# ChenFengTsai/dreamerv3-torch

Hardware: AMD Instinct MI355X
Metric: imagination-steps/sec (higher is better)
Workload: dtype f32; 1 GPU; cfg2: dmc_vision 64x64x3 synthetic replay, RSSM deter=512 hidden=512 stoch=32x32, continuous actor (6), imag_gradient dynamics, batch 16 x seq 64 per GPU, horizon 15; one step = full Dreamer._train update (world model + actor + critic fwd/bwd, gradient all-reduce, 3x clip+Adam); global_batch=16, seq_len=64, horizon=15, parallelism=dp1

## Files before the change

dreamerv3-torch_amd/csrc/fusedops.hip:

```cpp
#include "dv3_common.h"

namespace dv3 {

typedef float f32x4 __attribute__((ext_vector_type(4)));
typedef float f32x4u __attribute__((ext_vector_type(4), aligned(4)));

struct OLParams {
  const int* idx;
  int S, D;
  const float* x2;
  long ldx2;
  int A2;
  const float* WT;
  long ldw;
  const float* base;
  long ldbase;
  float* pre;
  long ldpre;
  const float* gamma;
  const float* beta;
  float* y;
  long ldy;
  float* mean;
  float* rstd;
// ... 195 lines not shown
      const float d = p.pre[r * p.ldpre + c] - mean;
      q += d * d;
    }
    const float rstd = rsqrtf(block_sum_256(q, red) * inv_n + kLnEps);
    for (int c = tid; c < p.N; c += 256) {
      const float t = (p.pre[r * p.ldpre + c] - mean) * rstd * p.gamma[c] + p.beta[c];
      p.y[r * p.ldy + c] = p.act ? siluf_(t) : t;
    }
    if (tid == 0) {
      if (p.mean) p.mean[r] = mean;
      if (p.rstd) p.rstd[r] = rstd;
    }
  }
}

struct AHParams {
  const float* pre;
  long ldpre;
  const float* gamma;
  const float* beta;
  float* y;
  long ldy;
  float* mean;
  float* rstd;
  const float* Wm;
  const float* bm;
  const float* Ws;
  const float* bs;
  float* out_m;
  float* out_s;
// ... 273 lines not shown
      ldpre < N || (base && ldbase < N))
    return DV3_ERR_ARG;
  if (y && (!gamma || !beta || ldy < N)) return DV3_ERR_ARG;
  OLParams p{idx, S, D, x2, ldx2, A2, WT, ldw, base, ldbase, pre, ldpre, gamma, beta, y, ldy, mean, rstd, M, N, act};
  hipStream_t s = (hipStream_t)stream;
  const bool vec = (N % 256 == 0) && N <= 1024 && (ldw % 4 == 0) && (ldpre % 4 == 0) && (!base || ldbase % 4 == 0) &&
                   (!y || ldy % 4 == 0);
  if (vec) {
    const dim3 grid(cap_grid(M, 1, 32768)), block(256);
    switch (N / 256) {
      case 1: hipLaunchKernelGGL((onehot_linear_ln_vec_kernel<1>), grid, block, 0, s, p); break;
      case 2: hipLaunchKernelGGL((onehot_linear_ln_vec_kernel<2>), grid, block, 0, s, p); break;
      case 3: hipLaunchKernelGGL((onehot_linear_ln_vec_kernel<3>), grid, block, 0, s, p); break;
      default: hipLaunchKernelGGL((onehot_linear_ln_vec_kernel<4>), grid, block, 0, s, p); break;
    }
  } else {
    hipLaunchKernelGGL(onehot_linear_ln_generic_kernel, dim3(cap_grid(M, 1, 16384)), dim3(256), 0, s, p);
  }
  return (int)hipGetLastError();
}

extern "C" int dv3_onehot_sample_linear_ln_fwd(const float* logit, const float* noise,
                                               const unsigned long long* rng_state, unsigned long long rng_offset,
                                               float* onehot, int* idx, const int* forced, unsigned int* flips,
                                               float unimix, int mode, const float* next_first, const float* init,
                                               const int* init_idx, float* next_out, int* next_idx, int S,
                                               const float* x2, long ldx2, int A2, const float* WT, long ldw,
                                               float* pre, long ldpre, const float* gamma, const float* beta, float* y,
                                               long ldy, float* mean, float* rstd, long M, int N, int act,
                                               void* stream) {
// ... 94 lines not shown
```

dreamerv3-torch_amd/dv3hip/engine.py:

```python
from __future__ import annotations

from dataclasses import dataclass
from typing import Dict, List, Optional

import torch

from . import _dev, ops

F32 = torch.float32


_FUSE_BLEND = _dev.flag("DV3_FUSE_BLEND", True)
_FUSE_SAMPLE = _dev.flag("DV3_FUSE_SAMPLE", True)
_GATHER_OBS = _dev.flag("DV3_GATHER_OBS", True)
_FUSE_SAMPLE_IN = _dev.flag("DV3_FUSE_SAMPLE_IN", True)
_FUSE_CARRY = _dev.flag("DV3_FUSE_CARRY", True)
_FUSE_SCAN_ROW = _dev.flag("DV3_FUSE_SCAN_ROW", True)
_FUSE_SCAN_LN = _dev.flag("DV3_FUSE_SCAN_LN", True)
_FUSE_SCAN_LNBWD = _dev.flag("DV3_FUSE_SCAN_LNBWD", True)
_FUSE_SCAN_CS = _dev.flag("DV3_FUSE_SCAN_CS", True)
_DEFER_CONV_WGRAD = _dev.flag("DV3_DEFER_CONV_WGRAD", True)
_FUSE_SCAN_GRUBWD = _dev.flag("DV3_FUSE_SCAN_GRUBWD", True)


class Lanes:

    _by_dev: Dict[str, "Lanes"] = {}

    @classmethod
    def get(cls, device):
        key = str(torch.device(device))
        if key not in cls._by_dev:
            try:
                cls._by_dev[key] = Lanes(device, _dev.value("DV3_LANES_SCAN_CUS", 0))
            except (RuntimeError, ValueError) as e:
                import sys

# ... 328 lines not shown

def v2(t: torch.Tensor, cols: int) -> torch.Tensor:
    return t.reshape(-1, cols)


def dense_ln_fwd(L: PDenseLN, x1, x2, pre, mean, rstd, y, *, accumulate_pre=False):
    ops.gemm(x1, L.W, pre, A2=x2, accumulate=accumulate_pre)
    ops.ln_act_fwd(pre, L.g, L.b, y, mean, rstd, act=True)


def dense_ln_bwd_pre(L: PDenseLN, dy, pre, mean, rstd, dpre, *, wgrad: bool):
    ops.ln_act_bwd(dy, pre, L.g, L.b, mean, rstd, dpre, _g(L.g) if wgrad else None, _g(L.b) if wgrad else None,
                   act=True)


def lin_wgrad(W, dY, x1, x2=None):
    k1 = x1.shape[1]
    gW = _g(W)
    ops.gemm(dY, x1, gW[:, :k1] if x2 is not None else gW, transA=True, transB=False, accumulate=True)
    if x2 is not None:
        ops.gemm(dY, x2, gW[:, k1:], transA=True, transB=False, accumulate=True)


class MLPEngine:

    def __init__(self, name: str, P: PMLP, ws: Workspace):
        self.name, self.P, self.ws = name, P, ws
        self.total = 0

    def _bufs(self, total):
        P, ws, nm = self.P, self.ws, self.name
        self.total = total
        acts = []
        for i, L in enumerate(P.layers):
# ... 49 lines not shown
                           None if onehot else out2[rs], head["action"], head["ent"], noise=head.get("noise"),
                           rng=head.get("rng"), eps_out=head.get("eps_out"), act_idx=head.get("act_idx"),
                           forced=head.get("forced"), flips=head.get("flips"), min_std=head.get("min_std", 0.1),
                           max_std=head.get("max_std", 1.0), unimix=head.get("unimix", 0.01), onehot=onehot)
            return h1, out[rs], None if onehot else out2[rs]
        o = o2 = None
        if out is not None:
            o = out[rs]
            ops.gemm(h1, P.out.W, o, A2=h2, bias=P.out.b)
        if out2 is not None:
            o2 = out2[rs]
            ops.gemm(h1, P.out2.W, o2, bias=P.out2.b)
        return h1, o, o2

    def backward(self, x1, x2, rows: slice, dout=None, dout2=None, *, wgrad: bool, dx1=None, dx2=None,
                 acc_dx=False, dh=None, defer=None):
        P, ws, nm = self.P, self.ws, self.name
        acts, _, _ = self._bufs(self.total)
        R = x1.shape[0]
        n_layers = len(P.layers)
        h = acts[-1][3][rows] if n_layers else x1
        first = True
        if dh is not None:
            first = False
        else:
            dh = ws.get(f"{nm}.dh", (R, h.shape[1]))
        for lin, d in ((P.out, dout), (P.out2, dout2)):
            if lin is None or d is None:
                continue
            ops.gemm(d, lin.W, dh, transB=False, accumulate=not first)
            first = False
# ... 1 lines not shown
                def _head_wgrad(lin=lin, d=d, h=h):
                    lin_wgrad(lin.W, d, h)
                    if lin.b is not None:
                        ops.colsum(d, _g(lin.b), accumulate=True)
                (defer.append if defer is not None else (lambda f: f()))(_head_wgrad)
        if first:
            raise ValueError("MLP backward without any upstream gradient")
        dy = dh
        for i in reversed(range(n_layers)):
            L = P.layers[i]
            pre, mean, rstd, _ = acts[i]
            xin1, xin2 = (acts[i - 1][3][rows], None) if i > 0 else (x1, x2)
            dpre = ws.get(f"{nm}.dpre{i}", (R, pre.shape[1]))
            dense_ln_bwd_pre(L, dy, pre[rows], mean[rows], rstd[rows], dpre, wgrad=wgrad)
            if wgrad:
                def _wg(L=L, dpre=dpre, xin1=xin1, xin2=xin2):
                    lin_wgrad(L.W, dpre, xin1, xin2)
                (defer.append if defer is not None else (lambda f: f()))(_wg)
            if i > 0:
                dprev = ws.get(f"{nm}.dy{i - 1}", (R, xin1.shape[1]))
                ops.gemm(dpre, L.W, dprev, transB=False)
                dy = dprev
            else:
                k1 = x1.shape[1]
                if dx1 is not None:
                    ops.gemm(dpre, L.W[:, :k1] if x2 is not None else L.W, dx1, transB=False, accumulate=acc_dx)
                if dx2 is not None and x2 is not None:
                    ops.gemm(dpre, L.W[:, k1:], dx2, transB=False, accumulate=acc_dx)


def _scan_bandwidth_bound(De: int, Hd: int, B: int) -> bool:
    gru_weight_bytes = 4 * 3 * De * (Hd + De)
# ... 279 lines not shown
                                      gd[t - 1] if t > 0 else None, dstoch0, ddeter0)
        side.join()
        ops.gemm(v2(dx3pre, Hd), P.obs_out.W[:, De:], v2(dembed, E), transB=False)
        dpl = v2(dpl_out, SW)

        def _scan_wgrads():
            if prior_inline:
                _prior_wgrads()
            lin_wgrad(P.obs.W, dpl, v2(x3, Hd))
            ops.colsum(dpl, _g(P.obs.b), accumulate=True)
            lin_wgrad(P.obs_out.W, v2(dx3pre, Hd), v2(deter, De), v2(self._embed, E))
            lin_wgrad(P.gru.W, v2(dgpre, 3 * De), v2(x1, Hd), v2(din, De))
            lin_wgrad(P.img_in.W, v2(dx1pre, Hd), v2(sin, SD), v2(ain, A))
            self.init_state_bwd(dstoch0, ddeter0)

        side.run([_scan_wgrads], chain=False)
        return side

    def pack_img_in(self, defer=None, name="rssm.img_in_wt"):
        W = self.P.img_in.W
        wt = self.ws.get(name, (W.shape[1], W.shape[0]))
        if defer is not None:
            defer.append((W, wt))
        else:
            ops.transpose2d(W, wt)
        return wt

    def img_step_fwd(self, stoch, deter, action, bufs, *, noise=None, rng=None, sample=True, forced=None,
                     flips=None, idx=None, idx_out=None, wcat=None, head=True):
        P = self.P
        M = stoch.shape[0]
# ... 152 lines not shown
            ops.ln_act_bwd(dy if last else dy.view(R, Co), pre.view(R, Co), L.g, L.b, mean, rstd, dpre.view(R, Co),
                           _g(L.g), _g(L.b), act=True, chw_group=OH * OH if last else 0)
            ops.conv_s2_wgrad(dpre, x, _g(L.W))
            if i > 0:
                wpt = ws.get(f"enc.wpt{i}", (4, Ci, 4 * Co))
                ops.pack_conv_weight(L.W, wpt, transposed=True)
                dx = ws.get(f"enc.dy{i - 1}", x.shape)
                ops.convT_s2_fwd(dpre, wpt, dx, Ci=Co, Co=Ci)
                dy = dx


class ConvDecoderEngine:
    def __init__(self, lin: PLin, layers: List[PConvLayer], ws: Workspace, minres=4):
        self.lin, self.L, self.ws, self.minres = lin, layers, ws, minres

    def forward(self, x1, x2):
        ws = self.ws
        R = x1.shape[0]
        E = self.lin.W.shape[0]
        mr = self.minres
        C0 = E // (mr * mr)
        h0 = ws.get("dec.h0", (R, mr, mr, C0))
        ops.gemm(x1, self.lin.W, h0.view(R, E), A2=x2, bias=self.lin.b)
        self._x = (x1, x2)
        self._acts = []
        x, H = h0, mr
        for i, L in enumerate(self.L):
            Ci, Co = L.W.shape[0], L.W.shape[1]
            OH = 2 * H
            c3 = L.g is None and Co == 3 and Ci in ops.C3_WIDTHS
            if not c3:
                wpt = ws.get(f"dec.wpt{i}", (4, Co, 4 * Ci))
                ops.pack_conv_weight(L.W, wpt, transposed=True)
            if L.g is not None:
                pre = ws.get(f"dec.pre{i}", (R, OH, OH, Co))
                ops.convT_s2_fwd(x, wpt, pre, Ci=Ci, Co=Co)
                rows = R * OH * OH
                mean, rstd = ws.get(f"dec.m{i}", (rows,)), ws.get(f"dec.r{i}", (rows,))
# ... 30 lines not shown
                    run(lambda dpre=dpre, L=L, rows=rows, Co=Co: ops.colsum(dpre.view(rows, Co), _g(L.bias),
                                                                         accumulate=True))
            (run if _DEFER_CONV_WGRAD else (lambda f: f()))(lambda x=x, dpre=dpre, L=L: ops.conv_s2_wgrad(x, dpre, _g(L.W)))
            dx = ws.get(f"dec.dx{i}", x.shape)
            if Co == 3 and Ci in ops.C3_WIDTHS:
                ops.conv_s2_c3_fwd(dpre, L.W, dx, CW=Ci)
            else:
                wp = ws.get(f"dec.wp{i}", (Ci, 16 * Co))
                ops.pack_conv_weight(L.W, wp, transposed=False)
                ops.conv_s2_fwd(dpre, wp, dx, Ci=Co, Co=Ci)
            dy = dx
        R = dy.shape[0]
        E = self.lin.W.shape[0]
        dh0 = dy.view(R, E)
        x1, x2 = self._x

        def _lin_wg():
            lin_wgrad(self.lin.W, dh0, x1, x2)
            ops.colsum(dh0, _g(self.lin.b), accumulate=True)

        run(_lin_wg)
        k1 = x1.shape[1]
        ops.gemm(dh0, self.lin.W[:, :k1], dx1, transB=False, accumulate=acc_dx)
        ops.gemm(dh0, self.lin.W[:, k1:], dx2, transB=False, accumulate=acc_dx)


class EnsembleEngine:

    def __init__(self, name: str, bucket, layers: int, ws: Workspace, *, std: float, scale: float = 1.0, log: bool = True):
        if bucket.members < 2 or layers < 1:
            raise ValueError("EnsembleEngine: needs at least 2 members (the unbiased std) and 1 trunk layer")
        self.name, self.bucket, self.L, self.ws = name, bucket, int(layers), ws
        self.K = bucket.members
# ... 102 lines not shown
```

dreamerv3-torch_amd/dv3hip/graph.py:

```python
from __future__ import annotations

from typing import Dict

import numpy as np
import torch

from . import _dev, _lib, ops


class CaptureRefused(RuntimeError):
    """The HIP runtime (or torch) refused stream capture / graph instantiation.  The ONLY condition under which the
    runners fall back to eager launches; shape bugs, a non-zero return code of a dv3 kernel (DV3Error) or an
    asynchronous HIP fault propagate to the caller."""


_CAPTURE_REFUSALS = (
    "hiperrorstreamcapture", "cudaerrorstreamcapture", "hiperrorcapturedevent", "hiperrorgraphexecupdatefailure",
    "operation not permitted when stream is capturing", "operation failed due to a previous error during capture",
    "operation would result in a merge of separate capture sequences",
    "capture was not ended in the same stream as it began", "capturing stream has unjoined work",
    "dependency created on uncaptured work in another stream",
    "operation would make the legacy stream depend on a capturing blocking stream",
    "operation not permitted on an event last recorded in a capturing stream",
    "attempt to terminate a thread-local capture sequence from another thread",
# ... 141 lines not shown
    @staticmethod
    def _launch(g, stream, lane, trace):
        if trace is None:
            g.replay()
            return
        a, b = torch.cuda.Event(enable_timing=True), torch.cuda.Event(enable_timing=True)
        a.record(stream)
        g.replay()
        b.record(stream)
        trace.append((lane, a, b))


_PIPE_PLAN = dict(on=_dev.flag("DV3_PIPE", True), a_split=_dev.value("DV3_PIPE_A_SPLIT", 0) or None,
                  c_split=_dev.value("DV3_PIPE_C_SPLIT", 0) or None, defer=_dev.value("DV3_PIPE_DEFER", "auto", str),
                  late=_dev.flag("DV3_PIPE_LATE", True), mode=_dev.value("DV3_PIPE_MODE", "auto", str),
                  defer_split=_dev.value("DV3_PIPE_DEFER_SPLIT", 0) or None)


class PhaseRecorder:

    def __init__(self, pool, device, lanes, lane_of, first_label, optional=()):
        self.pool, self.device, self.lanes = pool, device, lanes
        self.lane_of, self.first, self.optional = lane_of, first_label, set(optional)
        self.segments = []
        self._cur = None

    def _begin(self, label):
        g = torch.cuda.CUDAGraph()
        kw = dict(pool=self.pool, capture_error_mode="thread_local")
        lane = self.lane_of(label)
        if lane != "main":
# ... 355 lines not shown
        wm, beh = self.wm, self.beh
        dev = next(iter(self._static.values())).device
        lanes = engine.Lanes.get(dev)
        plan = self.pipe_plan
        rng_wm, rng_beh = ops.PhasedRng(dev), ops.PhasedRng(dev)
        key_dev = wm.dynamics.W.device
        lane_wm = lambda lb: {"wm.fscan": "scan", "wm.fscan2": "scan", "wm.rscan": "scan", "wm.rscan2": "scan",
                              "wm.defer": "side"}.get(lb, "main")
        lane_beh = lambda lb: "side" if lb.startswith(("bh.A", "bh.C")) else "main"
        mode = self._pipe_mode()
        if plan.get("defer", "auto") == "auto":
            plan["defer"] = "post" if wm._config.imag_gradient in ("dynamics", "both") else "side"
        if mode == "staged" and plan["defer"] != "side":
            lane_wm = lambda lb: {"wm.fscan": "scan", "wm.fscan2": "scan", "wm.rscan": "scan", "wm.rscan2": "scan"}.get(lb, "main")
        if mode == "lanes":
            lane_wm = lambda lb: "side" if lb == "wm.defer" else "scan"
            lane_beh = lambda lb: "side"
        opt_cuts = [f"bh.A@{plan['a_split']}"] if plan.get("a_split") else []
        opt_cuts += [f"bh.C@{plan['c_split']}"] if plan.get("c_split") else []
        cap = {}
        pool_w, pool_b = torch.cuda.graph_pool_handle(), torch.cuda.graph_pool_handle()
        w_cuts = [f"wm.defer@{plan['defer_split']}"] if (plan.get("defer_split") and mode == "lanes") else []
        with tools.rng_override(key_dev, rng_wm):
            W = PhaseRecorder(pool_w, dev, lanes, lane_wm, "wm.pre", optional=w_cuts).record(
                lambda: wm.train_fwd_bwd(self._static), at_end=rng_wm.finish_phase)
            gw = torch.cuda.CUDAGraph()

            def wopt():
                cap["post"], cap["ctx"], cap["m1"] = wm.train_opt(allreduce=False)

            _capture(gw, wopt, pool=pool_w)
        with tools.rng_override(key_dev, rng_beh):
            B = PhaseRecorder(pool_b, dev, lanes, lane_beh, "bh.start", optional=opt_cuts).record(
                lambda: beh.train_fwd_bwd(cap["post"]), at_end=rng_beh.finish_phase)
            gb = torch.cuda.CUDAGraph()
            _capture(gb, lambda: cap.update(beh_out=beh.train_opt(allreduce=False)), pool=pool_b)
        stride = rng_wm.taken + rng_beh.taken
        rng_wm.stride.fill_(stride), rng_beh.stride.fill_(stride)
        mk = lambda: torch.cuda.Event(blocking=True)
        self._pipe = dict(W=W.segments, B=B.segments, wopt=gw, bopt=gb, cap=cap, rng_wm=rng_wm, rng_beh=rng_beh,
                          lanes=lanes, entered=False, shared=tools.default_rng(key_dev), mode=mode,
                          ev={k: mk() for k in ("tail", "fork1", "q1", "mid", "fork2", "q2")},
                          ev2={k: (mk() if k == "mid" else torch.cuda.Event()) for k in ("load", "start", "mid", "defer", "wopt")},
                          ring=[mk(), mk()])

    def _pipe_enter(self):
        P = self._pipe
        sh = P["shared"]
        sh.commit()
        P["rng_beh"].state.copy_(sh.state)
        P["rng_wm"].state.copy_(sh.state)
        P["rng_wm"].state[1:2].add_(P["rng_beh"].taken)
        P["entered"] = True

    def _pipe_leave(self):
        P = self._pipe
        if P.get("lanes_running"):
            cur = torch.cuda.current_stream()
# ... 25 lines not shown
            ev["mid"].synchronize()
        self._load(data)
        ev["load"].record(cur)
        X.wait_event(ev["load"])
        if first:
            Y.wait_event(ev["load"])
        else:
            Y.wait_event(ev["wopt"])
        run(B, ["bh.start"], Y)
        ev["start"].record(Y)
        run(W, ["wm.pre"], X)
        run(B, [lb for lb in B if lb != "bh.start"], Y)
        X.wait_event(ev["start"])
        run(W, ["wm.fscan", "wm.fscan2", "wm.mid"], X)
        ev["mid"].record(X)
        run(W, ["wm.rscan", "wm.rscan2", "wm.post"] + [lb for lb in W if lb.startswith("wm.defer@")], X)
        with torch.cuda.stream(Y):
            self.beh._actor_opt.bucket.allreduce()
            self.beh._value_opt.bucket.allreduce()
            self._traced("bh.opt", P["bopt"])
            self._sink(1, P["cap"]["beh_out"][-1])
        Y.wait_event(ev["mid"])
        run(W, ["wm.defer"], Y)
        ev["defer"].record(Y)
        X.wait_event(ev["defer"])
        with torch.cuda.stream(X):
            self.wm._model_opt.bucket.allreduce()
            self._traced("wm.opt", P["wopt"])
            self._sink(0, P["cap"]["m1"])
        ev["wopt"].record(X)
        ring[it % 2].record(X)
        P["lanes_running"] = True

    def _traced(self, label, g):
        trace = self._pipe_trace
        if trace is None:
            g.replay()
            return
# ... 276 lines not shown
```

dreamerv3-torch_amd/dv3hip/ops.py:

```python
from __future__ import annotations

from typing import Optional

import torch

from . import _dev, _lib

F32 = torch.float32


def _stream() -> int:
    return torch.cuda.current_stream().cuda_stream


def _ptr(t: Optional[torch.Tensor]) -> int:
    return 0 if t is None else t.data_ptr()


def _f32(t: torch.Tensor, name: str) -> None:
    if not isinstance(t, torch.Tensor) or not t.is_cuda or t.dtype != F32:
        raise TypeError(f"{name}: expected a CUDA/HIP float32 tensor, got "
                        f"{type(t).__name__} {getattr(t, 'dtype', None)} {getattr(t, 'device', None)}")


# ... 1503 lines not shown
        _contig(gamma, "gamma"), _contig(beta, "beta")
        if (My, Ny) != (M, N) or gamma.numel() != N or beta.numel() != N:
            raise ValueError("y / LN affine shape mismatch")
        for t, nm in ((mean, "mean"), (rstd, "rstd")):
            if t is not None:
                _contig(t, nm)
                if t.numel() != M:
                    raise ValueError(nm + " size mismatch")
    _call("dv3_onehot_linear_ln_fwd", _ptr(idx), S, int(D), _ptr(x2), ldx2, A2, _ptr(WT), ldw, _ptr(base), ldbase,
          _ptr(pre), ldpre, _ptr(gamma), _ptr(beta), _ptr(y), ldy, _ptr(mean), _ptr(rstd), M, N, int(act), _stream(),
          key="dv3_onehot_linear_ln_fwd" + (f"[{M}x{N},S={S}]" if PROFILE.by_shape else ""),
          flops=2.0 * M * N * (S * D + A2), nbytes=4.0 * M * N * (S + 2))
    return y if y is not None else pre


def sample_linear_ln_ok(S, D, N) -> bool:
    return D == 32 and S <= 32 and N % 256 == 0 and N <= 1024


def onehot_sample_linear_ln(logit, out, *, next_first, init, init_idx, next_out, next_idx, WT, x2, pre, gamma, beta, y,
                            mean, rstd, noise=None, rng=None, idx=None, forced=None, flips=None, unimix=0.01,
                            mode=False, act=True):
    if logit.dim() != 3 or logit.shape[2] != 32:
        raise ValueError("logit must be [M,S,32]")
    M, S, D = logit.shape
    Kw, N, ldw = _rows2d(WT, "WT")
    Mp, Np, ldpre = _rows2d(pre, "pre")
    My, Ny, ldy = _rows2d(y, "y")
    Mx, A2, ldx2 = _rows2d(x2, "x2") if x2 is not None else (M, 0, 0)
    if not sample_linear_ln_ok(S, D, N) or (Mp, Np) != (M, N) or (My, Ny) != (M, N) or Mx != M or Kw != S * D + A2:
# ... 312 lines not shown
```

dreamerv3-torch_amd/models.py:

```python
from __future__ import annotations

import copy

import numpy as np
import torch
from torch import nn

import networks
import tools
from dv3hip import _dev
from dv3hip import engine as E
from dv3hip import ops
from dv3hip.params import ParamBucket

to_np = lambda x: x.detach().cpu().numpy()
_FUSED_IMAG = _dev.flag("DV3_FUSED_IMAG", True)
_STACK_DETER = _dev.flag("DV3_STACK_DETER", True)


import weakref

_BEHAVIORS = weakref.WeakKeyDictionary()
_RUNNERS = weakref.WeakKeyDictionary()

# ... 205 lines not shown
            ops.gauss_kl_fwd(out["post_mean"], out["post_std"], out["prior_mean"], out["prior_std"], kl, ent_p, ent_q)
        else:
            ops.kl_fwd(out["post_logit"], out["prior_logit"], kl, ent_p, ent_q, unimix=dyn._unimix_ratio)
        lanes_pay = rssm.lanes_pay(heavy_side=bool(self.heads["decoder"].cnn_shapes))
        E.SideStream.host_sync_point(lanes_pay)

        up = 1.0 / TB
        dec = self.heads["decoder"]
        acc = ws.zeros("wm.acc", (8 + len(dec.mlp_shapes),))
        gs, gd = ws.get("wm.gs", (T, B, SD)), ws.get("wm.gd", (T, B, De))
        wrote = False
        deferred = []
        grad_heads = cfg.grad_heads
        if dec.cnn_shapes:
            dec_eng = dec._cnn.engine
            recon = dec_eng.forward(ps, dt)
            limg = ws.get("wm.loss_img", (TB,))
            drecon = ws.get("wm.drecon", recon.shape)
            ops.mse_image(recon, st["image"], limg, drecon, upstream=up, perm=(B, T))
            ops.dot_accumulate(limg, acc[1:2], scale=up)
            dec_eng.backward(drecon, gs.view(TB, SD), gd.view(TB, De), acc_dx=False, defer=deferred)
            self._defer_heads_from = len(deferred)
            wrote = True
            if "decoder" not in grad_heads:
                gs.zero_(), gd.zero_()
        if dec.mlp_shapes:
            mdec = dec._mlp
            deng = mdec.engine_for(".wm")
            h, _, _ = deng.forward(ps, dt)
            dh = ws.zeros("wm.dec_dh", h.shape)
            for ki, (k, shp) in enumerate(dec.mlp_shapes.items()):
# ... 520 lines not shown
                       mix=getattr(cfg, "imag_gradient_mix", 0.0))
        R = H1N

        def _critic():
            inv = 1.0 / H1N
            up_v = ops.scale_neg(weights.view(HN)[:R], g("bh.up_v", (R,)), inv)
            lp, lp2 = g("bh.lp_v", (R,)), g("bh.lp_v2", (R,))
            dvl = g("bh.dv_logits", (R, 255))
            ops.disc_logprob_fwd(v_logits[:R], target.view(R), lp)
            ops.dot_accumulate(lp, acc[1:2], w=up_v)
            ops.disc_logprob_bwd(v_logits[:R], target.view(R), up_v, dvl)
            if cfg.critic["slow_target"]:
                ops.disc_logprob_fwd(v_logits[:R], slow.view(R), lp2)
                ops.dot_accumulate(lp2, acc[1:2], w=up_v)
                ops.disc_logprob_bwd(v_logits[:R], slow.view(R), up_v, dvl, accumulate=True)
            veng.backward(fs[:R], fd[:R], slice(0, R), dout=dvl, wgrad=True)

        E.Cuts.mark("bh.B@critic")
        side = E.SideStream(fs.device)
        side.run([_critic], chain=False)
        E.Cuts.mark("bh.B@dyn")
        daction = g("bh.daction", (H, N, A))
        if not reinforce:
            dreward, dcl = g("bh.dreward", (H, N)), g("bh.dcont", (H, N))
            ops.lambda_return_bwd(dtarget, value, c_logit.view(H, N), target, dreward, dcl, gamma=cfg.discount,
                                  lam=cfg.discount_lambda)
            gs, gd = g("bh.gs", (H, N, SD)), g("bh.gd", (H, N, De))
            rows = slice(N, HN)
            g_act = None
            if ens is not None:
                gs.view(HN, SD)[rows].zero_()
# ... 39 lines not shown
                ops.axpby(g_act.reshape(H, N, A).contiguous(), daction, 1.0, 1.0)
                R = HN
        dmean, dstd = g("bh.dmean", (R, A)), g("bh.dstd", (R, A))
        if normal:
            ops.actor_normal_bwd(a_mean[:R], a_std[:R], dmean, dstd, eps=im["eps"].view(HN, A)[:R],
                                 action=action.view(HN, A)[:R], daction=None if reinforce else daction.view(HN, A)[:R],
                                 dent=dent.view(HN)[:R], dlogp=dlogp.view(HN)[:R] if use_logp else None,
                                 min_std=cfg.actor["min_std"], max_std=cfg.actor["max_std"], logp_of_sample=use_logp)
        else:
            if not reinforce:
                ops.onehot_st_bwd(a_mean[:R], daction.view(HN, A)[:R], dmean, unimix=cfg.actor["unimix_ratio"])
            ops.onehot_ent_logp_bwd(a_mean[:R], action.view(HN, A)[:R], dent.view(HN)[:R],
                                    dlogp.view(HN)[:R] if use_logp else None, dmean,
                                    unimix=cfg.actor["unimix_ratio"], accumulate=not reinforce)
            dstd = None
        im["actor"].backward(fs[:R], fd[:R], slice(0, R), dout=dmean, dout2=dstd, wgrad=True)
        side.join()
        ops.dot_accumulate(ent.view(HN), acc[2:3], scale=1.0 / HN)
        metrics = {}
        groups = [(value[:-1], "value", None, None), (target, "target", None, None), (reward, "imag_reward", None, None),
                  (action if normal else torch.argmax(action, dim=-1).float(), "imag_action", None, None)]
        if cfg.imag_gradient == "both":
            metrics["imag_gradient_mix"] = cfg.imag_gradient_mix
        if cfg.reward_EMA:
            scale = torch.clip(ema[1:2] - ema[0:1], min=1.0)
            groups.append((target, "normed_target", ema[0:1], scale))
            metrics["EMA_005"], metrics["EMA_095"] = ema[0], ema[1]
        metrics.update(tools.tensorstats_many(groups))
        metrics["actor_entropy"] = acc[2]
        self.ema_to_wire()
        self._last = dict(reward=reward, value=value, target=target, weights=weights, disc=disc, slow=slow)
# ... 8 lines not shown
```

include/dv3hip.h:

```cpp
#ifndef DV3HIP_H_
#define DV3HIP_H_

#ifdef __cplusplus
extern "C" {
#endif

#define DV3_ERR_ARG 10001

int dv3_version(void);
int dv3_dev_switches(void);

int dv3_gemm_f32(int transA, int transB, int M, int N, int K, const float* A, long lda, const float* A2,
                 long lda2, int K1, const float* B, long ldb, float* C, long ldc, const float* bias,
                 int accumulate, int tile, void* stream);

int dv3_gemm_split_f32(int M, int N, int K, const float* A, long lda, const float* B, long ldb, float* C, long ldc,
                       int accumulate, float* C2, long ldc2, int nsplit, int accumulate2, void* stream);

int dv3_gemm_tn_grouped_f32(int n, const float* const* A, const long* lda, const float* const* B, const long* ldb,
                            float* const* C, const long* ldc, const int* M, const int* N, const int* K,
                            const int* accumulate, void* stream);

int dv3_gemm_sample_f32(int M, int N, int K, const float* A, long lda, const float* A2, long lda2, int K1,
                        const float* B, long ldb, float* C, long ldc, const float* bias, const float* noise,
// ... 193 lines not shown

int dv3_onehot_linear_ln_fwd(const int* idx, int S, int D, const float* x2, long ldx2, int A2, const float* WT,
                             long ldw, const float* base, long ldbase, float* pre, long ldpre, const float* gamma,
                             const float* beta, float* y, long ldy, float* mean, float* rstd, long M, int N, int act,
                             void* stream);
int dv3_actor_head_fwd(const float* pre, long ldpre, const float* gamma, const float* beta, float* y, long ldy,
                       float* mean, float* rstd, const float* Wm, const float* bm, const float* Ws, const float* bs,
                       float* out_m, float* out_s, const float* noise, const unsigned long long* rng_state,
                       unsigned long long rng_offset, float* eps_out, float* action, float* entropy, int* act_idx,
                       const int* forced, unsigned int* flips, long M, int U, int A, float min_std, float max_std,
                       float unimix, int onehot, void* stream);
int dv3_transpose2d(const float* src, long lds, int R, int C, float* dst, long ldd, void* stream);
int dv3_transpose2d_many(int njobs, const unsigned long long* jobs_host, void* stream);
int dv3_onehot_to_idx(const float* onehot, int* idx, long R, int D, void* stream);

int dv3_ens_gemm_f32(int members, int transA, int transB, int M, int N, int K, const float* A, long lda,
                     long strideA, const float* B, long ldb, long strideB, float* C, long ldc, long strideC,
                     const float* bias, long strideBias, int accumulate, void* stream);
int dv3_ens_ln_act_fwd(const float* x, long ldx, const float* gamma, const float* beta, long strideG, float* y,
                       long ldy, float* mean, float* rstd, int members, int M, int N, void* stream);
int dv3_ens_ln_act_bwd(const float* dy, long lddy, const float* x, long ldx, const float* gamma, const float* beta,
                       long strideG, const float* mean, const float* rstd, float* dx, long lddx, float* dgamma,
                       float* dbeta, int members, int M, int N, void* stream);
int dv3_ens_colsum(const float* x, long ldx, long strideX, float* out, long strideOut, int members, int M, int N,
                   int accumulate, void* stream);
int dv3_ens_regress_loss(const float* pre, const float* target, long ldt, float* dpre, float* loss, float* ws,
                         int members, int M, int W, float std, void* stream);
int dv3_ens_disag_fwd(const float* h, long ldh, long strideH, const float* w, long ldw, long strideW,
                      const float* bias, long strideBias, float* mu, float* part, float* disag, float* reward,
                      long ldr, int members, int M, int W, int U, float scale, int use_log, void* stream);
// ... 12 lines not shown
```

Before: 1.187 million imagination-steps/s.

## Use sparse one-hot kernels for decoder linear and actor/critic weight gradients

Adds a kernel that computes weight gradients for one-hot stochastic inputs by scatter-adding dY rows into per-category LDS bins, with a row-chunked fold. The dense GEMM over a mostly-zero one-hot matrix goes away. The decoder's first linear layer now uses a gathered one-hot forward through a new wide kernel plus a transposed weight copy. The pipeline also moves the RSSM scan weight-gradient segment to the side lane and sets the default defer split to 6. This brings extra workspace and a transpose, and the new paths are more complex.

```diff
diff --git a/dreamerv3-torch_amd/csrc/fusedops.hip b/dreamerv3-torch_amd/csrc/fusedops.hip
--- a/dreamerv3-torch_amd/csrc/fusedops.hip
+++ b/dreamerv3-torch_amd/csrc/fusedops.hip
@@ -233,6 +233,31 @@
   }
 }
 
+__global__ __launch_bounds__(256) void onehot_linear_wide_kernel(OLParams p) {
+  const int c = blockIdx.y * 1024 + 4 * threadIdx.x;
+  if (c >= p.N) return;
+  constexpr int MAXB = 16;
+  for (long r = blockIdx.x; r < p.M; r += gridDim.x) {
+    f32x4 acc = (f32x4){0.f, 0.f, 0.f, 0.f};
+    if (p.base) acc = *reinterpret_cast<const f32x4u*>(p.base + r * p.ldbase + c);
+    for (int s0 = 0; s0 < p.S; s0 += MAXB) {
+      f32x4 t[MAXB];
+#pragma unroll
+      for (int u = 0; u < MAXB; ++u) {
+        const int s = s0 + u;
+        t[u] = (f32x4){0.f, 0.f, 0.f, 0.f};
+        if (s < p.S) t[u] = *reinterpret_cast<const f32x4u*>(p.WT + (long)(s * p.D + p.idx[r * p.S + s]) * p.ldw + c);
+      }
+#pragma unroll
+      for (int u = 0; u < MAXB; ++u)
+        if (s0 + u < p.S) acc += t[u];
+    }
+    for (int a = 0; a < p.A2; ++a)
+      acc += p.x2[r * p.ldx2 + a] * *reinterpret_cast<const f32x4u*>(p.WT + (long)(p.S * p.D + a) * p.ldw + c);
+    *reinterpret_cast<f32x4u*>(p.pre + r * p.ldpre + c) = acc;
+  }
+}
+
 struct AHParams {
   const float* pre;
   long ldpre;
@@ -536,6 +561,9 @@
       case 3: hipLaunchKernelGGL((onehot_linear_ln_vec_kernel<3>), grid, block, 0, s, p); break;
       default: hipLaunchKernelGGL((onehot_linear_ln_vec_kernel<4>), grid, block, 0, s, p); break;
     }
+  } else if (!y && N > 1024 && N % 4 == 0 && ldw % 4 == 0 && ldpre % 4 == 0 && (!base || ldbase % 4 == 0)) {
+    hipLaunchKernelGGL(onehot_linear_wide_kernel, dim3(cap_grid(M, 1, 16384), (unsigned)((N + 1023) / 1024)), dim3(256), 0,
+                       s, p);
   } else {
     hipLaunchKernelGGL(onehot_linear_ln_generic_kernel, dim3(cap_grid(M, 1, 16384)), dim3(256), 0, s, p);
   }
diff --git a/dreamerv3-torch_amd/csrc/onehotops.hip b/dreamerv3-torch_amd/csrc/onehotops.hip
--- /dev/null
+++ b/dreamerv3-torch_amd/csrc/onehotops.hip
@@ -0,0 +1,202 @@
+#include "dv3_common.h"
+
+namespace dv3 {
+
+typedef float f32x4 __attribute__((ext_vector_type(4)));
+
+constexpr int kOwGroups = 8;
+constexpr int kOwRowChunk = 1024;
+constexpr int kOwRows = 4;
+constexpr int kOwBatches = 8;
+
+struct OWParams {
+  const int* idx;
+  int S;
+  const float* dY;
+  long lddy;
+  float* out;
+  long ldo;
+  long chunk_stride;
+  long R;
+  int U;
+  int accumulate;
+};
+
+template <int CPT>
+__device__ __forceinline__ int ow_slot(int j, int d) {
+  return d * (64 * CPT) + ((j + d) & 63) * CPT;
+}
+
+template <int CPT>
+__global__ __launch_bounds__(256) void onehot_wgrad_kernel(OWParams p) {
+  typedef float VT __attribute__((ext_vector_type(CPT)));
+  constexpr int CW = 64 * CPT, GW = kOwGroups / 4, RU = kOwRows, PF = kOwBatches;
+  extern __shared__ __attribute__((aligned(16))) float ow_bins[];
+  const int wave = __builtin_amdgcn_readfirstlane(threadIdx.x >> 6), l = threadIdx.x & 63;
+  const int s0 = blockIdx.y * kOwGroups + wave * GW;
+  if (s0 >= p.S) return;
+  const int ng = (p.S - s0 < GW) ? p.S - s0 : GW;
+  float* mine = ow_bins + wave * GW * 32 * CW;
+  for (int i = l * 4; i < GW * 32 * CW; i += 256) *reinterpret_cast<f32x4*>(mine + i) = (f32x4){0.f, 0.f, 0.f, 0.f};
+  const long r0 = (long)blockIdx.z * kOwRowChunk;
+  const long r1 = (r0 + kOwRowChunk < p.R) ? r0 + kOwRowChunk : p.R;
+  const float* __restrict__ dy = p.dY + (long)blockIdx.x * CW + l * CPT;
+  const int* __restrict__ ix = p.idx + s0;
+
+  const int lk = (l & (RU * GW - 1)) / GW, lg = (l % GW < ng) ? l % GW : ng - 1;
+  const long nfull = (r1 - r0) / (RU * PF) * (RU * PF);
+  VT xq[PF][RU];
+  int iq[PF];
+  if (nfull > 0) {
+#pragma unroll
+    for (int b = 0; b < PF; ++b) {
+#pragma unroll
+      for (int k = 0; k < RU; ++k) xq[b][k] = *reinterpret_cast<const VT*>(dy + (r0 + b * RU + k) * p.lddy);
+      iq[b] = ix[(r0 + b * RU + lk) * p.S + lg];
+    }
+  }
+  long r = r0;
+  for (; r < r0 + nfull; r += RU * PF) {
+#pragma unroll
+    for (int b = 0; b < PF; ++b) {
+    VT x[RU];
+    int id[RU][GW];
+#pragma unroll
+    for (int k = 0; k < RU; ++k) {
+      x[k] = xq[b][k];
+#pragma unroll
+      for (int g = 0; g < GW; ++g) id[k][g] = __builtin_amdgcn_readlane(iq[b], k * GW + g) & 31;
+    }
+    {
+      const long rn = r + (long)(PF + b) * RU;
+#pragma unroll
+      for (int k = 0; k < RU; ++k) {
+        const long rr = (rn + k < r0 + nfull) ? rn + k : r0 + nfull - 1;
+        xq[b][k] = *reinterpret_cast<const VT*>(dy + rr * p.lddy);
+      }
+      const long ri = (rn + lk < r0 + nfull) ? rn + lk : r0 + nfull - 1;
+      iq[b] = ix[ri * p.S + lg];
+    }
+    __builtin_amdgcn_sched_barrier(0);
+    VT bv[GW][RU], v[GW][RU];
+#pragma unroll
+    for (int g = 0; g < GW; ++g)
+#pragma unroll
+      for (int k = 0; k < RU; ++k) bv[g][k] = *reinterpret_cast<const VT*>(mine + g * 32 * CW + ow_slot<CPT>(l, id[k][g]));
+#pragma unroll
+    for (int g = 0; g < GW; ++g)
+#pragma unroll
+      for (int k = 0; k < RU; ++k) {
+        VT src = bv[g][k];
+#pragma unroll
+        for (int j = 0; j < k; ++j)
+          if (id[j][g] == id[k][g]) src = v[g][j];
+        v[g][k] = src + x[k];
+      }
+#pragma unroll
+    for (int g = 0; g < GW; ++g)
+#pragma unroll
+      for (int k = 0; k < RU; ++k) *reinterpret_cast<VT*>(mine + g * 32 * CW + ow_slot<CPT>(l, id[k][g])) = v[g][k];
+    __builtin_amdgcn_sched_barrier(0);
+    }
+  }
+  for (; r < r1; ++r) {
+    const VT xr = *reinterpret_cast<const VT*>(dy + r * p.lddy);
+    for (int g = 0; g < ng; ++g) {
+      VT* b = reinterpret_cast<VT*>(mine + g * 32 * CW + ow_slot<CPT>(l, ix[r * p.S + g] & 31));
+      *b = *b + xr;
+    }
+  }
+
+  float* out = p.out + (long)blockIdx.z * p.chunk_stride;
+  const int d = l & 31, h = l >> 5;
+  constexpr int WB = 16;
+  for (int g = 0; g < ng; ++g) {
+    const float* bin = mine + g * 32 * CW;
+    for (int c0 = h; c0 < CW; c0 += 2 * WB) {
+      float vsum[WB], old[WB];
+      float* o[WB];
+#pragma unroll
+      for (int j = 0; j < WB; ++j) {
+        const int c = c0 + 2 * j;
+        vsum[j] = bin[ow_slot<CPT>(c / CPT, d) + c % CPT];
+        o[j] = out + ((long)blockIdx.x * CW + c) * p.ldo + (long)(s0 + g) * 32 + d;
+        old[j] = 0.f;
+      }
+      if (p.accumulate) {
+#pragma unroll
+        for (int j = 0; j < WB; ++j) old[j] = *o[j];
+      }
+#pragma unroll
+      for (int j = 0; j < WB; ++j) *o[j] = old[j] + vsum[j];
+    }
+  }
+}
+
+__global__ __launch_bounds__(256) void onehot_wgrad_fold_kernel(const float* __restrict__ part, int chunks, long chunk_stride,
+                                                                float* gW, long ldw, int U, int SD, int accumulate) {
+  const long n = (long)U * SD;
+  for (long i = (long)blockIdx.x * 256 + threadIdx.x; i < n; i += (long)gridDim.x * 256) {
+    const long u = i / SD;
+    const int j = (int)(i - u * SD);
+    float* o = gW + u * ldw + j;
+    float acc = accumulate ? *o : 0.f;
+    for (int z = 0; z < chunks; ++z) acc += part[z * chunk_stride + i];
+    *o = acc;
+  }
+}
+
+static int ow_chunks(long R) { return (int)((R + kOwRowChunk - 1) / kOwRowChunk); }
+static bool ow_shape_ok(long R, int S, int D, int U) {
+  return D == 32 && S > 0 && U > 0 && U % 64 == 0 && R > 0 && ow_chunks(R) <= 65535 && (S + kOwGroups - 1) / kOwGroups <= 65535;
+}
+
+template <int CPT>
+static int ow_launch(const OWParams& p, dim3 grid, hipStream_t s) {
+  constexpr size_t lds = sizeof(float) * kOwGroups * 32 * 64 * CPT;
+  if (lds > 64 * 1024) {
+    static unsigned long long seen[4];
+    if (dv3_first_on_device(seen)) {
+      const hipError_t e = hipFuncSetAttribute(reinterpret_cast<const void*>(&onehot_wgrad_kernel<CPT>),
+                                               hipFuncAttributeMaxDynamicSharedMemorySize, (int)lds);
+      if (e != hipSuccess) return (int)e;
+    }
+  }
+  hipLaunchKernelGGL((onehot_wgrad_kernel<CPT>), grid, dim3(256), lds, s, p);
+  return (int)hipGetLastError();
+}
+
+}
+
+using namespace dv3;
+
+extern "C" int dv3_onehot_wgrad_row_chunk(void) { return kOwRowChunk; }
+
+extern "C" int dv3_onehot_wgrad_chunks(long R, int S, int D, int U) { return ow_shape_ok(R, S, D, U) ? ow_chunks(R) : 0; }
+
+extern "C" int dv3_onehot_wgrad_f32(const int* idx, int S, int D, const float* dY, long lddy, float* gW, long ldw, long R,
+                                    int U, int accumulate, float* ws, long ws_floats, void* stream) {
+  if (R <= 0) return 0;
+  if (!idx || !dY || !gW || D <= 0 || S <= 0 || U <= 0 || lddy < U || ldw < (long)S * D) return DV3_ERR_ARG;
+  if (!ow_shape_ok(R, S, D, U)) return DV3_ERR_ARG;
+  const int chunks = ow_chunks(R);
+  const long SD = (long)S * D, part = (long)U * SD;
+  if (chunks > 1 && (!ws || ws_floats < chunks * part)) return DV3_ERR_ARG;
+  hipStream_t s = (hipStream_t)stream;
+  OWParams p{idx, S, dY, lddy, gW, ldw, 0, R, U, accumulate ? 1 : 0};
+  if (chunks > 1) {
+    p.out = ws;
+    p.ldo = SD;
+    p.chunk_stride = part;
+    p.accumulate = 0;
+  }
+  const bool two = (U % 128 == 0) && (lddy % 2 == 0) && ((uintptr_t)dY % 8 == 0);
+  const dim3 grid((unsigned)(U / (two ? 128 : 64)), (unsigned)((S + kOwGroups - 1) / kOwGroups), (unsigned)chunks);
+  const int e = two ? ow_launch<2>(p, grid, s) : ow_launch<1>(p, grid, s);
+  if (e != 0 || chunks == 1) return e;
+  long blocks = (part + 255) / 256;
+  if (blocks > 16384) blocks = 16384;
+  hipLaunchKernelGGL(onehot_wgrad_fold_kernel, dim3((unsigned)blocks), dim3(256), 0, s, ws, chunks, part, gW, ldw, U,
+                     (int)SD, accumulate ? 1 : 0);
+  return (int)hipGetLastError();
+}
diff --git a/dreamerv3-torch_amd/dv3hip/engine.py b/dreamerv3-torch_amd/dv3hip/engine.py
--- a/dreamerv3-torch_amd/dv3hip/engine.py
+++ b/dreamerv3-torch_amd/dv3hip/engine.py
@@ -21,6 +21,7 @@
 _FUSE_SCAN_CS = _dev.flag("DV3_FUSE_SCAN_CS", True)
 _DEFER_CONV_WGRAD = _dev.flag("DV3_DEFER_CONV_WGRAD", True)
 _FUSE_SCAN_GRUBWD = _dev.flag("DV3_FUSE_SCAN_GRUBWD", True)
+_ONEHOT_WGRAD = _dev.flag("DV3_ONEHOT_WGRAD", True)
 
 
 class Lanes:
@@ -379,10 +380,14 @@
                    act=True)
 
 
-def lin_wgrad(W, dY, x1, x2=None):
+def lin_wgrad(W, dY, x1, x2=None, idx=None, D=0):
     k1 = x1.shape[1]
     gW = _g(W)
-    ops.gemm(dY, x1, gW[:, :k1] if x2 is not None else gW, transA=True, transB=False, accumulate=True)
+    g1 = gW[:, :k1] if x2 is not None else gW
+    if idx is not None and _ONEHOT_WGRAD and ops.onehot_wgrad_ok(idx.shape[0], idx.shape[1], D, dY.shape[1]):
+        ops.onehot_wgrad(idx, D, dY, g1, accumulate=True)
+    else:
+        ops.gemm(dY, x1, g1, transA=True, transB=False, accumulate=True)
     if x2 is not None:
         ops.gemm(dY, x2, gW[:, k1:], transA=True, transB=False, accumulate=True)
 
@@ -462,7 +467,7 @@
         return h1, o, o2
 
     def backward(self, x1, x2, rows: slice, dout=None, dout2=None, *, wgrad: bool, dx1=None, dx2=None,
-                 acc_dx=False, dh=None, defer=None):
+                 acc_dx=False, dh=None, defer=None, idx=None, D=0):
         P, ws, nm = self.P, self.ws, self.name
         acts, _, _ = self._bufs(self.total)
         R = x1.shape[0]
@@ -494,8 +499,8 @@
             dpre = ws.get(f"{nm}.dpre{i}", (R, pre.shape[1]))
             dense_ln_bwd_pre(L, dy, pre[rows], mean[rows], rstd[rows], dpre, wgrad=wgrad)
             if wgrad:
-                def _wg(L=L, dpre=dpre, xin1=xin1, xin2=xin2):
-                    lin_wgrad(L.W, dpre, xin1, xin2)
+                def _wg(L=L, dpre=dpre, xin1=xin1, xin2=xin2, idx=idx if i == 0 else None):
+                    lin_wgrad(L.W, dpre, xin1, xin2, idx, D)
                 (defer.append if defer is not None else (lambda f: f()))(_wg)
             if i > 0:
                 dprev = ws.get(f"{nm}.dy{i - 1}", (R, xin1.shape[1]))
@@ -805,7 +810,9 @@
             lin_wgrad(P.img_in.W, v2(dx1pre, Hd), v2(sin, SD), v2(ain, A))
             self.init_state_bwd(dstoch0, ddeter0)
 
+        Cuts.mark("wm.swg@side")
         side.run([_scan_wgrads], chain=False)
+        Cuts.mark("wm.post@enc")
         return side
 
     def pack_img_in(self, defer=None, name="rssm.img_in_wt"):
@@ -988,14 +995,31 @@
     def __init__(self, lin: PLin, layers: List[PConvLayer], ws: Workspace, minres=4):
         self.lin, self.L, self.ws, self.minres = lin, layers, ws, minres
 
-    def forward(self, x1, x2):
+    def pack_onehot(self, SD: int, defer=None):
+        W = self.lin.W
+        wt = self.ws.get("dec.wt", (SD, W.shape[0]))
+        if defer is not None:
+            defer.append((W[:, :SD], wt))
+        else:
+            ops.transpose2d(W[:, :SD], wt)
+        return wt
+
+    def forward(self, x1, x2, idx=None, D=0):
         ws = self.ws
         R = x1.shape[0]
         E = self.lin.W.shape[0]
         mr = self.minres
         C0 = E // (mr * mr)
         h0 = ws.get("dec.h0", (R, mr, mr, C0))
-        ops.gemm(x1, self.lin.W, h0.view(R, E), A2=x2, bias=self.lin.b)
+        if idx is not None and _ONEHOT_WGRAD:
+            SD = idx.shape[1] * D
+            hv = h0.view(R, E)
+            ops.gemm(x2, self.lin.W[:, SD:], hv, bias=self.lin.b)
+            ops.onehot_linear_ln(idx, D, ws.get("dec.wt", (SD, E)), hv, base=hv)
+        else:
+            idx = None
+            ops.gemm(x1, self.lin.W, h0.view(R, E), A2=x2, bias=self.lin.b)
+        self._idx = (idx, D)
         self._x = (x1, x2)
         self._acts = []
         x, H = h0, mr
@@ -1056,9 +1080,10 @@
         E = self.lin.W.shape[0]
         dh0 = dy.view(R, E)
         x1, x2 = self._x
+        idx, D = self._idx
 
         def _lin_wg():
-            lin_wgrad(self.lin.W, dh0, x1, x2)
+            lin_wgrad(self.lin.W, dh0, x1, x2, idx, D)
             ops.colsum(dh0, _g(self.lin.b), accumulate=True)
 
         run(_lin_wg)
diff --git a/dreamerv3-torch_amd/dv3hip/graph.py b/dreamerv3-torch_amd/dv3hip/graph.py
--- a/dreamerv3-torch_amd/dv3hip/graph.py
+++ b/dreamerv3-torch_amd/dv3hip/graph.py
@@ -179,7 +179,8 @@
 _PIPE_PLAN = dict(on=_dev.flag("DV3_PIPE", True), a_split=_dev.value("DV3_PIPE_A_SPLIT", 0) or None,
                   c_split=_dev.value("DV3_PIPE_C_SPLIT", 0) or None, defer=_dev.value("DV3_PIPE_DEFER", "auto", str),
                   late=_dev.flag("DV3_PIPE_LATE", True), mode=_dev.value("DV3_PIPE_MODE", "auto", str),
-                  defer_split=_dev.value("DV3_PIPE_DEFER_SPLIT", 0) or None)
+                  defer_split=_dev.value("DV3_PIPE_DEFER_SPLIT", 6) or None,
+                  scan_wgrads=_dev.value("DV3_PIPE_SCAN_WGRADS", "side", str))
 
 
 class PhaseRecorder:
@@ -565,13 +566,15 @@
         if mode == "staged" and plan["defer"] != "side":
             lane_wm = lambda lb: {"wm.fscan": "scan", "wm.fscan2": "scan", "wm.rscan": "scan", "wm.rscan2": "scan"}.get(lb, "main")
         if mode == "lanes":
-            lane_wm = lambda lb: "side" if lb == "wm.defer" else "scan"
+            lane_wm = lambda lb: "side" if lb in ("wm.defer", "wm.swg@side") else "scan"
             lane_beh = lambda lb: "side"
         opt_cuts = [f"bh.A@{plan['a_split']}"] if plan.get("a_split") else []
         opt_cuts += [f"bh.C@{plan['c_split']}"] if plan.get("c_split") else []
         cap = {}
         pool_w, pool_b = torch.cuda.graph_pool_handle(), torch.cuda.graph_pool_handle()
         w_cuts = [f"wm.defer@{plan['defer_split']}"] if (plan.get("defer_split") and mode == "lanes") else []
+        if mode == "lanes" and plan.get("scan_wgrads") == "side":
+            w_cuts += ["wm.swg@side", "wm.post@enc"]
         with tools.rng_override(key_dev, rng_wm):
             W = PhaseRecorder(pool_w, dev, lanes, lane_wm, "wm.pre", optional=w_cuts).record(
                 lambda: wm.train_fwd_bwd(self._static), at_end=rng_wm.finish_phase)
@@ -592,7 +595,7 @@
         self._pipe = dict(W=W.segments, B=B.segments, wopt=gw, bopt=gb, cap=cap, rng_wm=rng_wm, rng_beh=rng_beh,
                           lanes=lanes, entered=False, shared=tools.default_rng(key_dev), mode=mode,
                           ev={k: mk() for k in ("tail", "fork1", "q1", "mid", "fork2", "q2")},
-                          ev2={k: (mk() if k == "mid" else torch.cuda.Event()) for k in ("load", "start", "mid", "defer", "wopt")},
+                          ev2={k: (mk() if k == "mid" else torch.cuda.Event()) for k in ("load", "start", "mid", "swg", "defer", "wopt")},
                           ring=[mk(), mk()])
 
     def _pipe_enter(self):
@@ -648,7 +651,9 @@
         X.wait_event(ev["start"])
         run(W, ["wm.fscan", "wm.fscan2", "wm.mid"], X)
         ev["mid"].record(X)
-        run(W, ["wm.rscan", "wm.rscan2", "wm.post"] + [lb for lb in W if lb.startswith("wm.defer@")], X)
+        run(W, ["wm.rscan", "wm.rscan2", "wm.post"], X)
+        ev["swg"].record(X)
+        run(W, ["wm.post@enc"] + [lb for lb in W if lb.startswith("wm.defer@")], X)
         with torch.cuda.stream(Y):
             self.beh._actor_opt.bucket.allreduce()
             self.beh._value_opt.bucket.allreduce()
@@ -656,6 +661,9 @@
             self._sink(1, P["cap"]["beh_out"][-1])
         Y.wait_event(ev["mid"])
         run(W, ["wm.defer"], Y)
+        if "wm.swg@side" in W:
+            Y.wait_event(ev["swg"])
+            run(W, ["wm.swg@side"], Y)
         ev["defer"].record(Y)
         X.wait_event(ev["defer"])
         with torch.cuda.stream(X):
diff --git a/dreamerv3-torch_amd/dv3hip/ops.py b/dreamerv3-torch_amd/dv3hip/ops.py
--- a/dreamerv3-torch_amd/dv3hip/ops.py
+++ b/dreamerv3-torch_amd/dv3hip/ops.py
@@ -1541,6 +1541,39 @@
     return y if y is not None else pre
 
 
+_OW_WS = {}
+
+
+def onehot_wgrad_ok(R, S, D, U) -> bool:
+    return _lib.load().dv3_onehot_wgrad_chunks(int(R), int(S), int(D), int(U)) > 0
+
+
+def onehot_wgrad(idx, D, dY, gW, *, accumulate=True):
+    _contig(idx, "idx", torch.int32)
+    if idx.dim() != 2:
+        raise ValueError("idx must be [R,S]")
+    R, S = idx.shape
+    Ry, U, lddy = _rows2d(dY, "dY")
+    Ug, SD, ldw = _rows2d(gW, "gW")
+    if Ry != R or Ug != U or SD != S * D:
+        raise ValueError(f"onehot_wgrad: idx {tuple(idx.shape)} D {D} dY {tuple(dY.shape)} gW {tuple(gW.shape)}")
+    chunks = _lib.load().dv3_onehot_wgrad_chunks(R, S, int(D), U)
+    if chunks <= 0:
+        raise ValueError(f"onehot_wgrad: shape R {R} S {S} D {D} U {U} not taken (see onehot_wgrad_ok)")
+    ws, n = None, 0
+    s = _stream()
+    if chunks > 1:
+        n = chunks * U * SD
+        key = (n, str(dY.device), s)
+        ws = _OW_WS.get(key)
+        if ws is None:
+            ws = _OW_WS[key] = torch.empty(n, device=dY.device, dtype=F32)
+    _call("dv3_onehot_wgrad_f32", _ptr(idx), S, int(D), _ptr(dY), lddy, _ptr(gW), ldw, R, U, int(bool(accumulate)),
+          _ptr(ws), n, s, key="dv3_onehot_wgrad_f32" + (f"[{U}x{SD}x{R}]" if PROFILE.by_shape else ""),
+          flops=2.0 * R * U * SD, nbytes=4.0 * (R * U * -(-S // 8) + R * S + (2 * chunks + 1) * U * SD))
+    return gW
+
+
 def sample_linear_ln_ok(S, D, N) -> bool:
     return D == 32 and S <= 32 and N % 256 == 0 and N <= 1024
 
diff --git a/dreamerv3-torch_amd/models.py b/dreamerv3-torch_amd/models.py
--- a/dreamerv3-torch_amd/models.py
+++ b/dreamerv3-torch_amd/models.py
@@ -243,7 +243,10 @@
         grad_heads = cfg.grad_heads
         if dec.cnn_shapes:
             dec_eng = dec._cnn.engine
-            recon = dec_eng.forward(ps, dt)
+            didx = out["post_idx"].view(TB, S) if E._GATHER_OBS and not gauss else None
+            if didx is not None:
+                dec_eng.pack_onehot(SD)
+            recon = dec_eng.forward(ps, dt, idx=didx, D=D)
             limg = ws.get("wm.loss_img", (TB,))
             drecon = ws.get("wm.drecon", recon.shape)
             ops.mse_image(recon, st["image"], limg, drecon, upstream=up, perm=(B, T))
@@ -794,7 +797,7 @@
                 ops.disc_logprob_fwd(v_logits[:R], slow.view(R), lp2)
                 ops.dot_accumulate(lp2, acc[1:2], w=up_v)
                 ops.disc_logprob_bwd(v_logits[:R], slow.view(R), up_v, dvl, accumulate=True)
-            veng.backward(fs[:R], fd[:R], slice(0, R), dout=dvl, wgrad=True)
+            veng.backward(fs[:R], fd[:R], slice(0, R), dout=dvl, wgrad=True, idx=None if fidx is None else fidx[:R], D=D)
 
         E.Cuts.mark("bh.B@critic")
         side = E.SideStream(fs.device)
@@ -864,7 +867,8 @@
                                     dlogp.view(HN)[:R] if use_logp else None, dmean,
                                     unimix=cfg.actor["unimix_ratio"], accumulate=not reinforce)
             dstd = None
-        im["actor"].backward(fs[:R], fd[:R], slice(0, R), dout=dmean, dout2=dstd, wgrad=True)
+        im["actor"].backward(fs[:R], fd[:R], slice(0, R), dout=dmean, dout2=dstd, wgrad=True,
+                             idx=None if fidx is None else fidx[:R], D=D)
         side.join()
         ops.dot_accumulate(ent.view(HN), acc[2:3], scale=1.0 / HN)
         metrics = {}
diff --git a/include/dv3hip.h b/include/dv3hip.h
--- a/include/dv3hip.h
+++ b/include/dv3hip.h
@@ -231,6 +231,11 @@
 int dv3_transpose2d_many(int njobs, const unsigned long long* jobs_host, void* stream);
 int dv3_onehot_to_idx(const float* onehot, int* idx, long R, int D, void* stream);
 
+int dv3_onehot_wgrad_row_chunk(void);
+int dv3_onehot_wgrad_chunks(long R, int S, int D, int U);
+int dv3_onehot_wgrad_f32(const int* idx, int S, int D, const float* dY, long lddy, float* gW, long ldw, long R, int U,
+                         int accumulate, float* ws, long ws_floats, void* stream);
+
 int dv3_ens_gemm_f32(int members, int transA, int transB, int M, int N, int K, const float* A, long lda,
                      long strideA, const float* B, long ldb, long strideB, float* C, long ldc, long strideC,
                      const float* bias, long strideBias, int accumulate, void* stream);
```

Result: slower. 1.174 million imagination-steps/s (-1.0%).
